# shmurthy08/MoE-GAN_CPSC541

Hardware: AMD Instinct MI355X
Metric: images/sec (G+D step, 64x64 MS-COCO layout) (higher is better)
Workload: dtype bf16; 1 GPU; C2: 64x64, 8 experts top-2, batch 256/GPU, bf16, R1 on; global_batch=256, experts=8, topk=2, parallelism=dp1, world_seen=1, launch=hipGraph replay

## Files before the change

include/moegan_hip.h:

```cpp
#ifndef MOEGAN_HIP_H
#define MOEGAN_HIP_H
#include <stddef.h>
#include <stdint.h>

#ifdef __cplusplus
extern "C" {
#endif

#define MG_OK 0
#define MG_ERR_ARG (-1)
#define MG_ERR_LAUNCH (-2)

#define MG_F32 0
#define MG_BF16 1
#define MG_F32X3 2

#define MG_ACT_NONE 0
#define MG_ACT_LRELU 1
#define MG_ACT_GELU 2
#define MG_ACT_MUL_GELU_GRAD 3
#define MG_ACT_MUL_LRELU_GRAD 4
#define MG_ACT_RSQRT_EPS 5
#define MG_ACT_QUICK_GELU 6
#define MG_ACT_MUL_QUICK_GELU_GRAD 7
// ... 10 lines not shown
  int64_t ld_aux;
  const void* resid;
  int64_t ld_res;
  int32_t accumulate;
  int32_t atomic;
  int32_t remap_lgcin;
  int32_t remap_taps;
  const int32_t* a_idx;
  int32_t a_idx_div;
  const float* a_rowscale;
  int32_t a_gelu;
  const float* addvec;
  int32_t add_shift;
  int64_t add_ld;
  void* out_pre;
  int64_t ld_pre;
  float* gs;
  int64_t gs_ld;
  const void* gs_x;
  int64_t ld_gs_x;
} mg_epilogue;

const char* mg_last_error(void);
int mg_version(void);
const char* mg_source_hash(void);

int mg_set_workspace(void* ptr, size_t bytes, void* stream);
int mg_workspace_reserve(size_t bytes, void* stream);
int64_t mg_workspace_bytes(void* stream);
int mg_set_tuning(int key, int value);

int mg_timer_event_create(void** event);
int mg_timer_event_record(void* event, void* stream);
int mg_timer_event_elapsed(void* start, void* stop, float* ms);
int mg_timer_event_destroy(void* event);
int mg_mark(int tag, void* stream);

typedef struct mg_gemm_desc {
  int32_t M, N, K;
  const void* A;
  int64_t lda;
  const void* B;
  int64_t ldb;
  void* C;
  int64_t ldc;
  const mg_epilogue* ep;
} mg_gemm_desc;

int mg_gemm(int dtype, int M, int N, int K, const void* A, int64_t lda, int a_kc, const void* B, int64_t ldb,
            int b_kc, void* C, int64_t ldc, int c_dtype, const mg_epilogue* ep, int splits, void* stream);

int mg_gemm_batch(int dtype, int a_kc, int b_kc, int c_dtype, int n, const mg_gemm_desc* descs, void* stream);

int mg_conv2d_fwd(int dtype, const void* x, int B, int H, int W, int Cin, const void* wpack, int Cout, int KH,
                  int KW, int stride, int pad, const float* in_scale, void* y, int64_t ldy, int y_dtype,
                  const mg_epilogue* ep, void* stream);

int mg_conv2d_fwd_mx8(const void* x, const void* xscale, int B, int H, int W, int Cin, const void* wq,
                      const void* wscale, int Cout, int KH, int KW, int stride, int pad, void* y, int64_t ldy, int y_dtype, const mg_epilogue* ep,
                      void* stream);

int mg_quant_mx8(const void* x, int64_t ldx, int64_t rows, int K, void* q, void* scale, void* stream);
#define MG_QUANT_BATCH_MAX 32
typedef struct mg_quant_desc {
  const void* x;
  int64_t ldx;
  int64_t rows;
  int32_t K;
  void* q;
  void* scale;
} mg_quant_desc;
int mg_quant_mx8_batch(int n, const mg_quant_desc* d, void* stream);

int mg_conv2d_wgrad(int dtype, const void* gy, int64_t ldg, const void* x, int B, int H, int W, int Cin,
                    const float* in_scale, int Cout, int KH, int KW, int stride, int pad, float* gw, int splits,
                    void* stream);

int mg_conv2d_dgrad_s2(int dtype, const void* g, int B, int OH, int OW, int Cg, const void* wcls, int Cin,
                       void* out, int64_t ldo, int out_dtype, const mg_epilogue* ep, void* stream);

int mg_gemm_grouped(int dtype, int total_rows, int N, int K, int ngroups, const int32_t* row_off,
                    const int32_t* tile_off, int max_tiles, const void* A, int64_t lda, const void* B,
                    int64_t ldb, int b_kc, int64_t b_gstride, void* C, int64_t ldc, int c_dtype,
                    const mg_epilogue* ep, void* stream);

int mg_gemm_grouped_wgrad(int dtype, int M, int N, int ngroups, const int32_t* row_off, int total_rows,
                          const void* A, int64_t lda, const void* B, int64_t ldb, const int32_t* b_idx,
                          int b_idx_div, int b_gelu, float* C, int splits, const mg_epilogue* ep, void* stream);

int mg_moe_ffn_fwd(int dtype, int total_rows, int C, int Hd, int ngroups, const int32_t* row_off, const int32_t* tile_off, int max_tiles, const void* X, int64_t ldx, const int32_t* x_idx, int x_idx_div, const void* W1, const float* b1, const void* W2, const float* b2, void* pre, void* hid, void* Y, void* stream);

int mg_moe_ffn_bwd(int dtype, int total_rows, int C, int Hd, int ngroups, const int32_t* row_off, const int32_t* tile_off, int max_tiles, const void* gG, const void* pre, const void* W1, const void* W2, void* gP, void* gX, void* hid, float* gb1, float* gb2, void* stream);


int mg_clip_patches(int dtype, const void* img, int B, int R, int ld, int res, int patch, void* out, void* stream);

int mg_clip_patches_bwd(int g_dtype, const void* g_patches, int img_dtype, const void* img, int B, int R, int ld, int res, int patch, float alpha, int accumulate, void* g_img, void* stream);

int mg_cos_loss(const float* f, const float* text, int B, int C, const float* scale, float* loss, float* g_f, void* stream);

int mg_layernorm_fwd(int dtype, const void* x, int64_t ldx, int R, int C, const float* gamma, const float* beta, float eps, void* y, int64_t ldy, float* mean, float* rstd, int act, void* stream);

int mg_layernorm_bwd(int dtype, int gy_dtype, const void* gy, int64_t ldg, const void* x, int64_t ldx, int R, int C, const float* mean, const float* rstd, const float* gamma, void* gx, int64_t ldgx, int accumulate, float* ggamma, float* gbeta, void* stream);

int mg_attn_fwd(int dtype, const void* qkv, int B, int L, int C, int heads, void* out, float* lse, void* stream);

// ... 235 lines not shown
```

moe-gan_cpsc541_amd/csrc/mg_common.h:

```cpp
#pragma once
#include <hip/hip_runtime.h>
#include <stdint.h>

#include <algorithm>
#include <atomic>
#include <string>

#include "../../include/moegan_hip.h"

typedef uint16_t bf16_t;
typedef __bf16 bf16x8_t __attribute__((ext_vector_type(8)));
typedef unsigned short u16x8_t __attribute__((ext_vector_type(8)));
typedef unsigned short u16x4_t __attribute__((ext_vector_type(4)));
typedef float f32x4_t __attribute__((ext_vector_type(4)));

#define MG_DEV __device__ __forceinline__

MG_DEV float bf2f(bf16_t h) { return __uint_as_float(((uint32_t)h) << 16); }
MG_DEV bf16_t f2bf(float f) { return __builtin_bit_cast(bf16_t, (__bf16)f); }

MG_DEV float ldf(const float* p, int64_t i) { return p[i]; }
MG_DEV float ldf(const bf16_t* p, int64_t i) { return bf2f(p[i]); }
MG_DEV void stf(float* p, int64_t i, float v) { p[i] = v; }
MG_DEV void stf(bf16_t* p, int64_t i, float v) { p[i] = f2bf(v); }
// ... 76 lines not shown
  const V p = t * q;
  return gcopysign(gfma(-p, g, gsplat<V>(1.f)), x);
}
template <typename V> MG_DEV V gelu_fast_t(V x) {
  V g;
  const V e = gelu_erf_core(x, g);
  const V hx = x * gsplat<V>(0.5f);
  return gfma(hx, e, hx);
}
template <typename V> MG_DEV V gelu_fast_grad_t(V x) {
  V g;
  const V e = gelu_erf_core(x, g);
  return gfma(x * gsplat<V>(0.3989422804014327f), g, gfma(gsplat<V>(0.5f), e, gsplat<V>(0.5f)));
}
MG_DEV float gelu_fast(float x) { return gelu_fast_t<float>(x); }
MG_DEV float gelu_fast_grad(float x) { return gelu_fast_grad_t<float>(x); }
MG_DEV f32x2_t gelu_fast2(f32x2_t x) { return gelu_fast_t<f32x2_t>(x); }
MG_DEV f32x2_t gelu_fast_grad2(f32x2_t x) { return gelu_fast_grad_t<f32x2_t>(x); }

MG_DEV float wave_sum(float v) {
#pragma unroll
  for (int o = 32; o > 0; o >>= 1) v += __shfl_xor(v, o, 64);
  return v;
}
MG_DEV float wave_max(float v) {
#pragma unroll
  for (int o = 32; o > 0; o >>= 1) v = fmaxf(v, __shfl_xor(v, o, 64));
  return v;
}

void mg_set_error(const std::string& msg);
int mg_check_launch(const char* what);
enum { MG_TUNE_WGRAD_TILE = 0, MG_TUNE_GWGRAD_TILE = 1, MG_TUNE_CONV_TILE = 2, MG_TUNE_GEMM_TILE = 3,
       MG_TUNE_WGRAD_SPLITS = 4, MG_TUNE_NO_SLABS = 5, MG_TUNE_XCD = 6 , MG_TUNE_WGRAD_MODE = 7,
       MG_TUNE_WARP_LDS = 8, MG_TUNE_SHORTK = 9, MG_TUNE_ATOMIC_BLOCKS = 10, MG_TUNE_DETERMINISTIC = 11,
       MG_TUNE_S1_OFF = 12,
       MG_TUNE_D0_STORE = 13,
       MG_TUNE_FFN_BWD_OCC = 14,
       MG_TUNE_WIDE_WGRAD = 15,
       MG_TUNE_NARROW = 16,
       MG_TUNE_NARROW_BLOCKS = 17,
       MG_TUNE_DISPATCH3 = 18,
       MG_TUNE_NARROW_WPX = 19,
       MG_TUNE_GWGRAD_BLOCKS = 20,
       MG_TUNE_BATCH_SPLIT = 21,
       MG_TUNE_GROUPED_SHORTK = 22,
       MG_TUNE_SPLITK_FUSED = 23,
       MG_TUNE_ROUTER_TEAM = 24,
       MG_TUNE_ADAMW_CACHED = 25,
       MG_TUNE_ATOMIC_MINK = 26,
       MG_TUNE_WIDE_BLOCKS = 27,
       MG_TUNE_WGRAD_SLAB_BLOCKS = 28,
       MG_TUNE_MODGRAD_UNFUSED = 29,
       MG_TUNE_COUNT = 30 };
extern std::atomic<int> g_mg_tune[MG_TUNE_COUNT];
inline bool mg_det() { return g_mg_tune[MG_TUNE_DETERMINISTIC].load(std::memory_order_relaxed) != 0; }
void* mg_workspace(size_t bytes, hipStream_t stream);
int* mg_tile_counters(int n, hipStream_t stream);
void* mg_fold_alloc(size_t bytes, hipStream_t stream);
int mg_fold_rows_submit(const mg_fold_rows& r, bool deferred, hipStream_t stream);
int mg_fold_wgrad_submit(const mg_fold_wgrad& r, bool deferred, hipStream_t stream);
inline float* mg_fold_partials(size_t bytes, hipStream_t st, bool* deferred) {
  void* p = mg_fold_alloc(bytes, st);
  *deferred = p != nullptr;
  return reinterpret_cast<float*>(p ? p : mg_workspace(bytes, st));
}

namespace {
__global__ __launch_bounds__(1024) void k_det_fold_rows(const float* __restrict__ part, int nrows, int ncols, int na,
                                                        float* __restrict__ out_a, float* __restrict__ out_b) {
  __shared__ float red[16][64];
  const int cx = threadIdx.x & 63, ry = threadIdx.x >> 6;
  const int i = blockIdx.x * 64 + cx;
  float s = 0.f;
  if (i < ncols)
    for (int r = ry; r < nrows; r += 16) s += part[(int64_t)r * ncols + i];
  red[ry][cx] = s;
  __syncthreads();
  if (ry == 0 && i < ncols) {
    float t = 0.f;
#pragma unroll
    for (int y = 0; y < 16; ++y) t += red[y][cx];
    if (i < na) out_a[i] += t;
    else out_b[i - na] += t;
  }
}
__global__ __launch_bounds__(256) void k_det_sum(const float* __restrict__ part, int n, float* __restrict__ out) {
  __shared__ float ws[4];
  float s = 0.f;
  for (int i = threadIdx.x; i < n; i += blockDim.x) s += part[i];
#pragma unroll
  for (int o = 32; o > 0; o >>= 1) s += __shfl_xor(s, o, 64);
  if ((threadIdx.x & 63) == 0) ws[threadIdx.x >> 6] = s;
  __syncthreads();
  if (threadIdx.x == 0) out[0] += (ws[0] + ws[1]) + (ws[2] + ws[3]);
}
}
static inline void mg_det_fold_rows(const float* part, int nrows, int ncols, int na, float* out_a, float* out_b,
                             hipStream_t st) {
  hipLaunchKernelGGL(k_det_fold_rows, dim3((ncols + 63) / 64), dim3(1024), 0, st, part, nrows, ncols, na, out_a, out_b);
}

#define MG_REQUIRE(cond, msg)                       \
  do {                                              \
    if (!(cond)) {                                  \
      mg_set_error(std::string(__func__) + ": " + (msg)); \
      return MG_ERR_ARG;                            \
    }                                               \
  } while (0)

static inline int cdiv(int64_t a, int64_t b) { return (int)((a + b - 1) / b); }

bool mg_conv3_direct_ok(int H, int W, int Cin, int Cout, int KH, int KW, int stride, int pad, bool wgrad);
bool mg_conv3_direct(const void* x, int B, int H, int Cin, const void* wpack, int Cout, const mg_epilogue* e, void* y,
                     int64_t ldy, int y_dtype, hipStream_t st);
bool mg_wgrad3_direct(const void* gy, int64_t ldg, const void* x, int B, int H, int Cin, float** ws_out, int* splits,
                      bool* deferred,
                      hipStream_t st);

int mg_modgrad_gemm(int dtype, int M, int N, int K, const void* A, int64_t lda, const void* B, int64_t ldb, void* C,
                    int64_t ldc, int c_dtype, const mg_epilogue* e, hipStream_t st);
int mg_modgrad_conv(int dtype, const void* x, int B, int H, int W, int Cin, const void* wpack, int Cout, void* y,
                    int64_t ldy, int y_dtype, const mg_epilogue* e, hipStream_t st);

bool mg_wgrad_wide(int M, int N, int K, const void* A, int64_t lda, const void* B, int64_t ldb, float* C, int64_t ldc,
                   float alpha, hipStream_t st);
```

moe-gan_cpsc541_amd/csrc/mg_gemm.hip:

```cpp
#include <algorithm>
#include <string>
#include <type_traits>

#include "mg_gemm.h"
#include "mg_host.h"

using namespace mg;

namespace {


constexpr Grouping kNoGroup{0, 1, nullptr, nullptr, 0};
inline Grouping xcd_group() {
  Grouping g = kNoGroup;
  const int x = g_mg_tune[MG_TUNE_XCD];
  g.swz = x == 0 ? 1 : x == 3 ? 0 : x;
  return g;
}

inline bool a_xf(const mg_epilogue* e) { return e && (e->a_idx || e->a_rowscale || e->a_gelu); }

template <typename T, typename TO, int BM, int BN, bool AK, bool BKc, bool XF, bool X3 = false>
void run_plain(int M, int N, int K, const void* A, int64_t lda, const void* B, int64_t ldb, void* C, int64_t ldc,
               const mg_epilogue* e, int splits, hipStream_t st) {
// ... 113 lines not shown
                         grid, dim3(NTHREADS), 0, st, la, lb, slab, M, N, K, kchunk, xcd_group());
  };
  const T* Ap = reinterpret_cast<const T*>(A);
  const T* Bp = reinterpret_cast<const T*>(B);
  using TT = std::true_type;
  using FF = std::false_type;
  if (a_kc) {
    LdKC<T> la{Ap, lda, M, K, nullptr, 1, nullptr, 0};
    if (b_kc) go(la, LdKC<T>{Bp, ldb, N, K, nullptr, 1, nullptr, 0}, TT{}, TT{});
    else go(la, LdMC<T>{Bp, ldb, N, K, nullptr, 1, nullptr, 0}, TT{}, FF{});
  } else {
    LdMC<T> la{Ap, lda, M, K, nullptr, 1, nullptr, 0};
    if (b_kc) go(la, LdKC<T>{Bp, ldb, N, K, nullptr, 1, nullptr, 0}, FF{}, TT{});
    else go(la, LdMC<T>{Bp, ldb, N, K, nullptr, 1, nullptr, 0}, FF{}, FF{});
  }
  if (cnt) return true;
  int blocks = (int)std::min<int64_t>(cdiv(MN, 256), 2048);
  hipLaunchKernelGGL((splitk_reduce_kernel<Epi<TO>>), dim3(blocks), dim3(256), 0, st, ws, splits, M, N, ep);
  return true;
}

}

extern "C" int mg_gemm(int dtype, int M, int N, int K, const void* A, int64_t lda, int a_kc, const void* B,
                       int64_t ldb, int b_kc, void* C, int64_t ldc, int c_dtype, const mg_epilogue* ep, int splits,
                       void* stream) {
  MG_REQUIRE(dtype == MG_F32 || dtype == MG_BF16 || dtype == MG_F32X3, "bad dtype");
  MG_REQUIRE(M >= 0 && N >= 0 && K >= 0, "negative size");
  if (M == 0 || N == 0) return MG_OK;
  const bool qgg = ep && ep->act == MG_ACT_MUL_QUICK_GELU_GRAD;
  MG_REQUIRE(!qgg || (dtype == MG_BF16 && c_dtype == MG_BF16 && a_kc && !b_kc && splits <= 1 && ep->aux &&
                      !ep->bias && !ep->scale && !ep->out_pre && !ep->atomic && !ep->remap_taps && !a_xf(ep)),
             "MG_ACT_MUL_QUICK_GELU_GRAD: bf16 g [M,K] x W [K,N] -> bf16 with aux, no bias / scale / out_pre / atomic");
  const bool x3 = dtype == MG_F32X3;
  if (x3) dtype = MG_F32;
  const int vec = dtype == MG_F32 ? 4 : 8;
  MG_REQUIRE(aligned16(A) && aligned16(B), "A/B must be 16-byte aligned");
  MG_REQUIRE(lda % vec == 0 && ldb % vec == 0, "lda/ldb must be multiples of the 16-byte vector");
  MG_REQUIRE(a_kc ? (K % vec == 0) : (M % vec == 0), "A vector dim must be a multiple of the 16-byte vector");
  MG_REQUIRE(b_kc ? (K % vec == 0) : (N % vec == 0), "B vector dim must be a multiple of the 16-byte vector");
  MG_REQUIRE(under2g((a_kc ? (int64_t)M : K) * lda, dtype) && under2g((b_kc ? (int64_t)N : K) * ldb, dtype) &&
                 under2g((int64_t)M * ldc, c_dtype),
             "an operand exceeds 2 GiB (32-bit buffer offsets)");
  if (ep && ep->gs) {
    MG_REQUIRE(a_kc && !b_kc && !x3 && splits <= 1, "mg_epilogue.gs: gyt [M, K] x W [K, N], bf16 or fp32, no split-K");
    return mg_modgrad_gemm(dtype, M, N, K, A, lda, B, ldb, C, ldc, c_dtype, ep, reinterpret_cast<hipStream_t>(stream));
  }
  if (splits < 1 && dtype == MG_BF16 && !x3 && !a_kc && !b_kc && c_dtype == MG_F32 && ep && ep->atomic &&
      !ep->bias && !ep->scale && !ep->rowscale && !ep->act && !ep->aux && !ep->resid && !ep->accumulate &&
      !ep->remap_taps && !ep->a_idx && !ep->a_rowscale && !ep->a_gelu && !ep->addvec && !ep->out_pre &&
      mg_wgrad_wide(M, N, K, A, lda, B, ldb, reinterpret_cast<float*>(C), ldc, ep->alpha,
                    reinterpret_cast<hipStream_t>(stream)))
    return mg_check_launch("mg_gemm (wide weight gradient)");
  if (splits < 1) {
    if (ep && ep->atomic) {
      int64_t tiles = (int64_t)cdiv(M, 64) * cdiv(N, 64);
      const int target = g_mg_tune[MG_TUNE_ATOMIC_BLOCKS] > 0 ? (int)g_mg_tune[MG_TUNE_ATOMIC_BLOCKS] : 512;
      int64_t want = std::max<int64_t>(1, target / std::max<int64_t>(tiles, 1));
      const int mink = g_mg_tune[MG_TUNE_ATOMIC_MINK] > 0 ? (int)g_mg_tune[MG_TUNE_ATOMIC_MINK] : 256;
      splits = (int)std::max<int64_t>(1, std::min<int64_t>(want, K / mink));
    } else {
      splits = 1;
    }
  }
  MG_REQUIRE(splits == 1 || (ep && ep->atomic && c_dtype == MG_F32), "split-K requires an atomic fp32 epilogue");
  MG_REQUIRE(!(ep && ep->atomic) || c_dtype == MG_F32, "atomic epilogue requires fp32 C");
  if (K == 0) splits = 1;
  hipStream_t st = reinterpret_cast<hipStream_t>(stream);
  if (splits > 1 && mg_det()) {
    bool done;
    if (x3)
      done = run_splitk_slabs<float, float, true>(a_kc, b_kc, M, N, K, A, lda, B, ldb, C, ldc, ep, st, splits);
    else if (dtype == MG_F32)
      done = run_splitk_slabs<float, float>(a_kc, b_kc, M, N, K, A, lda, B, ldb, C, ldc, ep, st, splits);
    else
      done = run_splitk_slabs<bf16_t, float>(a_kc, b_kc, M, N, K, A, lda, B, ldb, C, ldc, ep, st, splits);
    if (done) return mg_check_launch("mg_gemm (deterministic split-K slabs)");
    splits = 1;
  }
  if (splits == 1 && !(ep && ep->atomic) && !qgg && !g_mg_tune[MG_TUNE_NO_SLABS]) {
    bool done;
    if (x3)
      done = c_dtype == MG_F32 ? run_splitk_slabs<float, float, true>(a_kc, b_kc, M, N, K, A, lda, B, ldb, C, ldc, ep, st)
                               : run_splitk_slabs<float, bf16_t, true>(a_kc, b_kc, M, N, K, A, lda, B, ldb, C, ldc, ep, st);
    else if (dtype == MG_F32)
      done = c_dtype == MG_F32 ? run_splitk_slabs<float, float>(a_kc, b_kc, M, N, K, A, lda, B, ldb, C, ldc, ep, st)
                               : run_splitk_slabs<float, bf16_t>(a_kc, b_kc, M, N, K, A, lda, B, ldb, C, ldc, ep, st);
    else
      done = c_dtype == MG_F32 ? run_splitk_slabs<bf16_t, float>(a_kc, b_kc, M, N, K, A, lda, B, ldb, C, ldc, ep, st)
                               : run_splitk_slabs<bf16_t, bf16_t>(a_kc, b_kc, M, N, K, A, lda, B, ldb, C, ldc, ep, st);
    if (done) return mg_check_launch("mg_gemm (split-K slabs)");
  }
  if (x3) {
    if (c_dtype == MG_F32) run_plain_tiles<float, float, true>(a_kc, b_kc, M, N, K, A, lda, B, ldb, C, ldc, ep, splits, st);
    else run_plain_tiles<float, bf16_t, true>(a_kc, b_kc, M, N, K, A, lda, B, ldb, C, ldc, ep, splits, st);
  } else if (dtype == MG_F32) {
    if (c_dtype == MG_F32) run_plain_tiles<float, float>(a_kc, b_kc, M, N, K, A, lda, B, ldb, C, ldc, ep, splits, st);
    else run_plain_tiles<float, bf16_t>(a_kc, b_kc, M, N, K, A, lda, B, ldb, C, ldc, ep, splits, st);
  } else {
    if (c_dtype == MG_F32) run_plain_tiles<bf16_t, float>(a_kc, b_kc, M, N, K, A, lda, B, ldb, C, ldc, ep, splits, st);
    else run_plain_tiles<bf16_t, bf16_t>(a_kc, b_kc, M, N, K, A, lda, B, ldb, C, ldc, ep, splits, st);
  }
  return mg_check_launch("mg_gemm");
}

namespace {
// ... 56 lines not shown
      r.n = used;
      float* ws = reinterpret_cast<float*>(mg_workspace((size_t)std::max<int64_t>(off, 8) * sizeof(float), st));
      if (ws) {
        args.ws = ws;
        r.ws = ws;
        hipLaunchKernelGGL((gemm_batch_kernel<T, AK, BKc, AL, BL, TO, X3, true>), dim3(tiles, S), dim3(NTHREADS), 0, st,
                           args);
        hipLaunchKernelGGL((batch_reduce_kernel<TO>), dim3(blks), dim3(256), 0, st, r);
        continue;
      }
    }
    hipLaunchKernelGGL((gemm_batch_kernel<T, AK, BKc, AL, BL, TO, X3>), dim3(tiles), dim3(NTHREADS), 0, st, args);
  }
  return mg_check_launch("mg_gemm_batch");
}
}

extern "C" int mg_gemm_batch(int dtype, int a_kc, int b_kc, int c_dtype, int n, const mg_gemm_desc* d,
                             void* stream) {
  MG_REQUIRE(dtype == MG_F32 || dtype == MG_BF16 || dtype == MG_F32X3, "bad dtype");
  const int vec = dtype == MG_BF16 ? 8 : 4;
  const int mdt = dtype == MG_F32X3 ? MG_F32 : dtype;
  for (int i = 0; i < n; ++i) {
    const mg_gemm_desc& q = d[i];
    MG_REQUIRE(q.M >= 0 && q.N >= 0 && q.K >= 0, "negative size");
    MG_REQUIRE(aligned16(q.A) && aligned16(q.B), "A/B must be 16-byte aligned");
    MG_REQUIRE(q.lda % vec == 0 && q.ldb % vec == 0, "lda/ldb must be multiples of the 16-byte vector");
    MG_REQUIRE(a_kc ? (q.K % vec == 0) : (q.M % vec == 0), "A vector dim must be a multiple of the vector");
    MG_REQUIRE(b_kc ? (q.K % vec == 0) : (q.N % vec == 0), "B vector dim must be a multiple of the vector");
    MG_REQUIRE(!(q.ep && q.ep->atomic) || c_dtype == MG_F32, "atomic epilogue requires fp32 C");
    MG_REQUIRE(!a_xf(q.ep), "A loader transforms (a_idx / a_rowscale / a_gelu) are not supported by mg_gemm_batch");
    MG_REQUIRE(!q.ep || q.ep->act != MG_ACT_MUL_QUICK_GELU_GRAD, "MG_ACT_MUL_QUICK_GELU_GRAD: mg_gemm only");
    MG_REQUIRE(under2g((a_kc ? (int64_t)q.M : q.K) * q.lda, mdt) &&
                   under2g((b_kc ? (int64_t)q.N : q.K) * q.ldb, mdt) && under2g((int64_t)q.M * q.ldc, c_dtype),
               "an operand exceeds 2 GiB (32-bit buffer offsets)");
  }
  if (n <= 0) return MG_OK;
  hipStream_t st = reinterpret_cast<hipStream_t>(stream);
  if (mg_det() && n > 1) {
    bool atomic = false;
    for (int i = 0; i < n; ++i) atomic = atomic || (d[i].ep && d[i].ep->atomic);
    if (atomic) {
      for (int i = 0; i < n; ++i) {
        int rc = mg_gemm_batch(dtype, a_kc, b_kc, c_dtype, 1, d + i, stream);
        if (rc) return rc;
      }
      return MG_OK;
    }
  }
#define B_(T, TO, ...)                                                                                          \
  (a_kc ? (b_kc ? run_batch<T, TO, true, true, ##__VA_ARGS__>(n, d, st) : run_batch<T, TO, true, false, ##__VA_ARGS__>(n, d, st)) \
        : (b_kc ? run_batch<T, TO, false, true, ##__VA_ARGS__>(n, d, st) : run_batch<T, TO, false, false, ##__VA_ARGS__>(n, d, st)))
  if (dtype == MG_F32) return c_dtype == MG_F32 ? B_(float, float) : B_(float, bf16_t);
  if (dtype == MG_F32X3) return c_dtype == MG_F32 ? B_(float, float, true) : B_(float, bf16_t, true);
  return c_dtype == MG_F32 ? B_(bf16_t, float) : B_(bf16_t, bf16_t);
#undef B_
}

namespace {
template <typename T, typename TO, int BM, int BN, bool XF = false, bool SC = false>
void run_conv(const void* x, int B, int H, int W, int Cin, const void* wpack, int Cout, int KH, int KW, int stride,
              int pad, const float* sc, void* y, int64_t ldy, const mg_epilogue* e, hipStream_t st) {
  int OH = (H + 2 * pad - KH) / stride + 1, OW = (W + 2 * pad - KW) / stride + 1;
  int M = B * OH * OW, K = KH * KW * Cin;
  LdKCConv<T, XF, SC> la{reinterpret_cast<const T*>(x), H, W, Cin, ilog2(Cin), ilog2(OW), ilog2(OH * OW), M,
                         KW, stride, pad, K, sc, kwinv(KW)};
  LdKC<T> lb{reinterpret_cast<const T*>(wpack), K, Cout, K, nullptr, 1, nullptr, 0};
  auto ep = make_epi<TO>(y, ldy, e);
  launch_gemm<T, BM, BN, true, true>(la, lb, ep, M, Cout, K, 1, kNoGroup, 0, st);
}
template <typename T, typename TO, bool SC, int BM, int BN>
bool conv_slabs_t(const void* x, int B, int H, int W, int Cin, const void* wpack, int Cout, int KH, int KW,
                  int stride, int pad, const float* sc, void* y, int64_t ldy, const mg_epilogue* e, hipStream_t st) {
  constexpr int TBK = tile_bk<T, false, BM, BN>();
  int OH = (H + 2 * pad - KH) / stride + 1, OW = (W + 2 * pad - KW) / stride + 1;
  int M = B * OH * OW, K = KH * KW * Cin;
  int64_t tiles = (int64_t)cdiv(M, BM) * cdiv(Cout, BN);
  const int ksteps = K / TBK;
  if (tiles >= 1024 || ksteps < 16 || (e && e->atomic) || sc || g_mg_tune[MG_TUNE_NO_SLABS]) return false;
  int splits = (int)std::min<int64_t>(cdiv(1024, tiles), ksteps / 8);
  if (splits < 2) return false;
  int kchunk = ((K + splits - 1) / splits + TBK - 1) / TBK * TBK;
  splits = (K + kchunk - 1) / kchunk;
  const int64_t MN = (int64_t)M * Cout;
  float* ws = reinterpret_cast<float*>(mg_workspace((size_t)splits * MN * sizeof(float), st));
  if (!ws) return false;
  mg_epilogue raw{};
  raw.alpha = 1.f;
  Epi<float> slab = make_epi<float>(ws, Cout, &raw);
  slab.zstride = MN;
  slab.vec_ok = slab.host_vec_ok() ? 1 : 0;
  LdKCConv<T, false, SC> la{reinterpret_cast<const T*>(x), H, W, Cin, ilog2(Cin), ilog2(OW), ilog2(OH * OW), M,
                            KW, stride, pad, K, sc, kwinv(KW)};
  LdKC<T> lb{reinterpret_cast<const T*>(wpack), K, Cout, K, nullptr, 1, nullptr, 0};
  dim3 grid(cdiv(M, BM), cdiv(Cout, BN), splits);
  auto ep = make_epi<TO>(y, ldy, e);
  ep.vec_ok = ep.host_vec_ok() ? 1 : 0;
  int* cnt = g_mg_tune[MG_TUNE_SPLITK_FUSED] == 1 ? mg_tile_counters((int)tiles, st) : nullptr;
  if (cnt) {
    hipLaunchKernelGGL((gemm_splitk_fused_kernel<T, BM, BN, true, true, LdKCConv<T, false, SC>, LdKC<T>, TO>), grid,
                       dim3(NTHREADS), 0, st, la, lb, slab, ep, M, Cout, K, kchunk, cnt);
    return true;
  }
  hipLaunchKernelGGL((gemm_kernel<T, BM, BN, true, true, LdKCConv<T, false, SC>, LdKC<T>, Epi<float>>), grid,
                     dim3(NTHREADS), 0, st, la, lb, slab, M, Cout, K, kchunk, xcd_group());
  int blocks = (int)std::min<int64_t>(cdiv(MN, 256), 2048);
// ... 417 lines not shown
```

moe-gan_cpsc541_amd/moegan_mi/roofline.py:

```python
import re

import torch

from . import _lib as L

ELT = {0: 4, 1: 2, 2: 4}
MX8_PEAK_TFLOPS = 5000.0

FAMILIES = {
    "conv_fwd": ("mfma", ("mg_conv2d_fwd",)),
    "conv_fwd_mx8": ("mfma8", ("mg_conv2d_fwd_mx8",)),
    "conv_dgrad_s2": ("mfma", ("mg_conv2d_dgrad_s2",)),
    "conv_wgrad+fold": ("mfma", ("mg_conv2d_wgrad",)),
    "expert_gemm": ("mfma", ("mg_gemm_grouped", "mg_gemm_grouped_wgrad", "mg_moe_ffn_fwd", "mg_moe_ffn_bwd")),
    "gemm": ("mfma", ("mg_gemm", "mg_gemm_batch")),
    "attention": ("mfma", ("mg_attn_fwd", "mg_attn_bwd", "mg_xattn_fwd", "mg_xattn_bwd", "mg_xattn_ragged_fwd",
                          "mg_xattn_ragged_bwd")),
    "router_fwd": ("hbm", ("mg_router_fwd",)),
    "dispatch_combine": ("hbm", ("mg_gather_rows", "mg_moe_combine")),
    "warp_fwd": ("hbm", ("mg_warp_fwd", "mg_warp_fwd_scaled")),
    "mtm_bwd": ("hbm", ("mg_mtm_bwd_fused",)),
    "modconv_bwd_io": ("hbm", ("mg_modconv_bwd_in", "mg_modconv_bwd_out", "mg_scale_bc")),
    "r1": ("hbm", ("mg_r1",)),
    "sumsq": ("hbm", ("mg_sumsq", "mg_grad_norm_steps")),
    "adamw": ("hbm", ("mg_adamw_dev", "mg_adamw_dev_shadow", "mg_adamw_dev_ema", "mg_adamw")),
    "bias_colsum": ("hbm", ("mg_colsum", "mg_grouped_colsum", "mg_colsum_batch", "mg_segsum", "mg_const_bwd")),
    "weight_prep": ("hbm", ("mg_pack_conv", "mg_pack_conv_flip", "mg_pack_dgrad_s2", "mg_wsq", "mg_wsq_bwd",
                            "mg_router_reparam", "mg_weight_norm_fwd", "mg_weight_norm_bwd", "mg_weight_norm_batch",
                            "mg_quant_mx8",
                            "mg_prep_batch")),
    "layernorm": ("hbm", ("mg_layernorm_fwd", "mg_layernorm_bwd")),
    "router_aux": ("hbm", ("mg_router_bwd", "mg_moe_gate_grad", "mg_moe_token_grad", "mg_router_feat_grad",
                           "mg_router_param_bwd", "mg_router_param_bwd_batch", "mg_moe_dispatch", "mg_router_kl",
                           "mg_router_kl_batch")),
    "im2col_col2im": ("hbm", ("mg_im2col_4x4s2", "mg_col2im_4x4s2")),
    "grad_fold": ("hbm", ("mg_fold_flush", "mg_fold_rows_batch", "mg_fold_rows_queue", "mg_fold_defer")),
    "d_conv0": ("hbm", ("mg_d0_fwd", "mg_d0_wgrad", "mg_d0_dgrad")),
    "elementwise": ("hbm", ("mg_cast", "mg_copy2d", "mg_lrelu_mask_mul", "mg_upsample2x_fwd", "mg_upsample2x_bwd",
                            "mg_const_fwd", "mg_gated_axpy", "mg_select_if", "mg_zero_if", "mg_clip_patches",
                            "mg_clip_patches_bwd")),
    "disc_head": ("hbm", ("mg_disc_head_fwd", "mg_disc_head_gmat", "mg_disc_head_sum", "mg_disc_head_bwd_data",
                          "mg_d_head_fwd", "mg_d_head_bwd",
                          "mg_disc_head_bwd_w", "mg_d_text_bwd")),
    "mtm_bwd_unfused": ("hbm", ("mg_warp_bwd", "mg_offset_head_bwd")),
    "losses_flags": ("hbm", ("mg_d_loss", "mg_g_loss", "mg_finite_flag", "mg_flag_window", "mg_kl_coefs", "mg_balance",
                             "mg_opt_prologue", "mg_guard_update", "mg_cos_loss")),
}
_FAMILY_OF = {e: f for f, (_, es) in FAMILIES.items() for e in es}

KERNELS = [
    (r"k_fold_wgrad_batch|k_fold_rows_batch", "grad_fold"),
    (r"k_wgrad_fold|splitk_reduce_kernel<mg::Epi<float>|k_wgrad3_direct", "conv_wgrad+fold"),
    (r"k_conv3_direct", "conv_fwd"),
    (r"k_mx8_conv", "conv_fwd_mx8"),
    (r"gemm_kernel<.*, 1(, (true|false))?>\(|k_moe_ffn_fwd|k_moe_ffn_bwd|k_ffn_bias_fold", "expert_gemm"),
    (r"gemm_kernel<[^>]*LdKCConvT", "conv_dgrad_s2"),
    (r"gemm_kernel<.*LdMCConv", "conv_wgrad+fold"),
    (r"gemm_kernel<.*LdKCConv", "conv_fwd"),
    (r"gemm_kernel<|gemm_batch_kernel<|splitk_reduce_kernel", "gemm"),
    (r"k_attn_|k_xattn_", "attention"),
    (r"k_router_fwd", "router_fwd"),
    (r"k_gather_rows|k_combine", "dispatch_combine"),
    (r"k_warp_fwd", "warp_fwd"),
    (r"k_mtm_bwd", "mtm_bwd"),
    (r"k_bwd_in|k_bwd_out|k_scale_bc", "modconv_bwd_io"),
    (r"k_r1", "r1"),
    (r"k_sumsq", "sumsq"),
    (r"k_adamw", "adamw"),
    (r"k_colsum|k_grouped_colsum|k_segsum|k_const_bwd", "bias_colsum"),
    (r"k_pack_|k_wsq|k_reparam|k_wn_|k_quant_mx8|k_prep_batch", "weight_prep"),
    (r"k_ln_|k_layernorm", "layernorm"),
    (r"k_router_bwd|k_fold_partials|k_gate_grad|k_token_grad|k_router_feat_grad|k_feat_grad_fin|k_router_param_bwd|"
     r"k_disp_|k_router_kl", "router_aux"),
    (r"k_im2col|k_col2im", "im2col_col2im"),
    (r"k_d0_|k_fold_cols", "d_conv0"),
    (r"k_wgrad_wide|k_wide_fold|k_wide_final", "gemm"),
    (r"k_cast|k_copy2d|k_mask_mul|k_up2|k_const_fwd|k_gated_axpy|k_select_if|k_zero_if|k_clip_patches",
     "elementwise"),
    (r"k_head_|k_d_text|k_dhead_", "disc_head"),
    (r"k_warp_bwd|k_offset_head", "mtm_bwd_unfused"),
    (r"k_d_loss|k_g_loss|k_finite_flag|k_flag_window|k_guard_update|k_kl_coefs|k_balance|k_opt_prologue|"
     r"k_cos_loss",
     "losses_flags"),
]


def kernel_family(kernel_name):
    for pat, fam in KERNELS:
        if re.search(pat, kernel_name):
            return fam
    return "other"


def _conv_out(H, W, KH, KW, s, p):
    return (H + 2 * p - KH) // s + 1, (W + 2 * p - KW) // s + 1


def work(name, a):
    if name in ("mg_conv2d_fwd", "mg_conv2d_wgrad", "mg_conv2d_fwd_mx8"):
        OH, OW = _conv_out(a["H"], a["W"], a["KH"], a["KW"], a["stride"], a["pad"])
        return 2.0 * a["B"] * OH * OW * a["Cout"] * a["KH"] * a["KW"] * a["Cin"]
    if name == "mg_conv2d_dgrad_s2":
        return 2.0 * a["B"] * (2 * a["OH"]) * (2 * a["OW"]) * a["Cin"] * a["Cg"] * 4
    if name == "mg_gemm":
        return 2.0 * a["M"] * a["N"] * a["K"]
    if name == "mg_gemm_batch":
        d = a["descs"]
        return sum(2.0 * d[i].M * d[i].N * d[i].K for i in range(a["n"]))
    if name == "mg_gemm_grouped":
        return 2.0 * a["total_rows"] * a["N"] * a["K"]
    if name == "mg_gemm_grouped_wgrad":
        return 2.0 * a["M"] * a["N"] * a["total_rows"]
# ... 359 lines not shown
```

Measured before the change: 32650 images/sec.

## Add small-M fp32x3 GEMM kernel with 32x32 tiles and in-block split-K

Adds a dedicated kernel for small fp32-emulated (bf16x3 split) GEMMs with M up to 512. It uses 32x32 tiles, a four-stage register prefetch pipeline, and waves that each take a slice of K and are reduced through shared memory. Both single and batched GEMM paths route to it when the shape and epilogue allow, with a tune flag to turn it off. The aim is more parallelism and less split-K reduction overhead on small router and head GEMMs. The cost is another code path whose epilogue support is limited, and it may lose to the existing tiled kernels on some shapes.

Result: no change. 32810 images/sec, median of 4 (+0.5%).

```diff
diff --git a/include/moegan_hip.h b/include/moegan_hip.h
--- a/include/moegan_hip.h
+++ b/include/moegan_hip.h
@@ -86,6 +86,8 @@
 
 int mg_gemm_batch(int dtype, int a_kc, int b_kc, int c_dtype, int n, const mg_gemm_desc* descs, void* stream);
 
+int mg_gemm_rows_fusable(int dtype, int M, int N, int K, const void* A, int64_t lda, int a_kc, const void* B, int64_t ldb, int b_kc, const void* C, int64_t ldc, int c_dtype, const mg_epilogue* ep, int splits);
+
 int mg_conv2d_fwd(int dtype, const void* x, int B, int H, int W, int Cin, const void* wpack, int Cout, int KH,
                   int KW, int stride, int pad, const float* in_scale, void* y, int64_t ldy, int y_dtype,
                   const mg_epilogue* ep, void* stream);
diff --git a/moe-gan_cpsc541_amd/csrc/mg_common.h b/moe-gan_cpsc541_amd/csrc/mg_common.h
--- a/moe-gan_cpsc541_amd/csrc/mg_common.h
+++ b/moe-gan_cpsc541_amd/csrc/mg_common.h
@@ -152,7 +152,8 @@
        MG_TUNE_WIDE_BLOCKS = 27,
        MG_TUNE_WGRAD_SLAB_BLOCKS = 28,
        MG_TUNE_MODGRAD_UNFUSED = 29,
-       MG_TUNE_COUNT = 30 };
+       MG_TUNE_ROWS_OFF = 30,
+       MG_TUNE_COUNT = 31 };
 extern std::atomic<int> g_mg_tune[MG_TUNE_COUNT];
 inline bool mg_det() { return g_mg_tune[MG_TUNE_DETERMINISTIC].load(std::memory_order_relaxed) != 0; }
 void* mg_workspace(size_t bytes, hipStream_t stream);
@@ -223,5 +224,8 @@
 int mg_modgrad_conv(int dtype, const void* x, int B, int H, int W, int Cin, const void* wpack, int Cout, void* y,
                     int64_t ldy, int y_dtype, const mg_epilogue* e, hipStream_t st);
 
+bool mg_rows_batch_ok(int dtype, int a_kc, int b_kc, int c_dtype, int n, const mg_gemm_desc* d);
+void mg_rows_launch(int b_kc, int c_dtype, int n, const mg_gemm_desc* d, bool batched, hipStream_t st);
+
 bool mg_wgrad_wide(int M, int N, int K, const void* A, int64_t lda, const void* B, int64_t ldb, float* C, int64_t ldc,
                    float alpha, hipStream_t st);
diff --git a/moe-gan_cpsc541_amd/csrc/mg_gemm.hip b/moe-gan_cpsc541_amd/csrc/mg_gemm.hip
--- a/moe-gan_cpsc541_amd/csrc/mg_gemm.hip
+++ b/moe-gan_cpsc541_amd/csrc/mg_gemm.hip
@@ -189,6 +189,11 @@
       mg_wgrad_wide(M, N, K, A, lda, B, ldb, reinterpret_cast<float*>(C), ldc, ep->alpha,
                     reinterpret_cast<hipStream_t>(stream)))
     return mg_check_launch("mg_gemm (wide weight gradient)");
+  if (x3 && mg_gemm_rows_fusable(MG_F32X3, M, N, K, A, lda, a_kc, B, ldb, b_kc, C, ldc, c_dtype, ep, splits)) {
+    const mg_gemm_desc q{M, N, K, A, lda, B, ldb, C, ldc, ep};
+    mg_rows_launch(b_kc, c_dtype, 1, &q, false, reinterpret_cast<hipStream_t>(stream));
+    return mg_check_launch("mg_gemm (batch rows)");
+  }
   if (splits < 1) {
     if (ep && ep->atomic) {
       int64_t tiles = (int64_t)cdiv(M, 64) * cdiv(N, 64);
@@ -351,6 +356,22 @@
   (a_kc ? (b_kc ? run_batch<T, TO, true, true, ##__VA_ARGS__>(n, d, st) : run_batch<T, TO, true, false, ##__VA_ARGS__>(n, d, st)) \
         : (b_kc ? run_batch<T, TO, false, true, ##__VA_ARGS__>(n, d, st) : run_batch<T, TO, false, false, ##__VA_ARGS__>(n, d, st)))
   if (dtype == MG_F32) return c_dtype == MG_F32 ? B_(float, float) : B_(float, bf16_t);
+  if (dtype == MG_F32X3 && a_kc && g_mg_tune[MG_TUNE_ROWS_OFF] != 1) {
+    for (int i0 = 0; i0 < n; i0 += MG_BATCH_MAX) {
+      const int cnt = std::min(MG_BATCH_MAX, n - i0);
+      const mg_gemm_desc* dc = d + i0;
+      if (mg_rows_batch_ok(dtype, a_kc, b_kc, c_dtype, cnt, dc)) {
+        mg_rows_launch(b_kc, c_dtype, cnt, dc, true, st);
+        continue;
+      }
+      const int rc = b_kc ? (c_dtype == MG_F32 ? run_batch<float, float, true, true, true>(cnt, dc, st)
+                                               : run_batch<float, bf16_t, true, true, true>(cnt, dc, st))
+                          : (c_dtype == MG_F32 ? run_batch<float, float, true, false, true>(cnt, dc, st)
+                                               : run_batch<float, bf16_t, true, false, true>(cnt, dc, st));
+      if (rc) return rc;
+    }
+    return mg_check_launch("mg_gemm_batch (batch rows)");
+  }
   if (dtype == MG_F32X3) return c_dtype == MG_F32 ? B_(float, float, true) : B_(float, bf16_t, true);
   return c_dtype == MG_F32 ? B_(bf16_t, float) : B_(bf16_t, bf16_t);
 #undef B_
diff --git a/moe-gan_cpsc541_amd/csrc/mg_rows.hip b/moe-gan_cpsc541_amd/csrc/mg_rows.hip
--- /dev/null
+++ b/moe-gan_cpsc541_amd/csrc/mg_rows.hip
@@ -0,0 +1,316 @@
+#include <algorithm>
+
+#include "mg_gemm.h"
+#include "mg_host.h"
+
+using namespace mg;
+
+namespace {
+
+constexpr int RW_BM = 32, RW_BN = 32;
+constexpr int RW_DEPTH = 4;
+constexpr int RW_MAXW = 8;
+constexpr int RW_PITCH = RW_BN + 4;
+constexpr int RW_MAX_M = 512;
+constexpr int64_t RW_MAX_WORK = (int64_t)1 << 27;
+
+template <typename TO>
+struct RowsArgs {
+  const float* A[MG_BATCH_MAX];
+  const float* B[MG_BATCH_MAX];
+  int64_t lda[MG_BATCH_MAX], ldb[MG_BATCH_MAX];
+  Epi<TO> e[MG_BATCH_MAX];
+  int M[MG_BATCH_MAX], N[MG_BATCH_MAX], K[MG_BATCH_MAX], tiles_m[MG_BATCH_MAX], tile_off[MG_BATCH_MAX + 1];
+  int per[MG_BATCH_MAX];
+  int n, total;
+};
+
+MG_DEV float bload1(rsrc_t r, uint32_t voff, uint32_t soff) {
+  return __builtin_bit_cast(float, __builtin_amdgcn_raw_buffer_load_b32(r, voff, soff, 0));
+}
+
+MG_DEV void split8(const float* v, bf16x8_t& hi, bf16x8_t& lo) {
+  u16x8_t h, l;
+#pragma unroll
+  for (int j = 0; j < 8; ++j) {
+    h[j] = f2bf(v[j]);
+    l[j] = f2bf(v[j] - bf2f(h[j]));
+  }
+  hi = __builtin_bit_cast(bf16x8_t, h);
+  lo = __builtin_bit_cast(bf16x8_t, l);
+}
+
+template <bool B_KC, typename TO>
+__global__ __launch_bounds__(RW_MAXW * 64) void gemm_rows_kernel(RowsArgs<TO> args) {
+  extern __shared__ __attribute__((aligned(16))) float rw_part[];
+  const int per8 = (args.total + 7) >> 3;
+  const int t = (blockIdx.x & 7) * per8 + (blockIdx.x >> 3);
+  if (t >= args.total) return;
+  int p = 0;
+  while (p + 1 < args.n && t >= args.tile_off[p + 1]) ++p;
+  const int lt = t - args.tile_off[p];
+  const int tn = lt / args.tiles_m[p], tm = lt - tn * args.tiles_m[p];
+  const int m0 = tm * RW_BM, n0 = tn * RW_BN;
+  const int M = args.M[p], N = args.N[p], K = args.K[p];
+  const int W = blockDim.x >> 6;
+  const int wave = __builtin_amdgcn_readfirstlane(threadIdx.x >> 6), lane = threadIdx.x & 63;
+  const int fq = lane >> 4, fr = lane & 15;
+
+  const int steps = (K + 31) >> 5, per = args.per[p];
+  const int s_beg = wave * per, s_end = min(steps, s_beg + per);
+  const int nact = min(W, (steps + per - 1) / per);
+
+  const rsrc_t rA = make_rsrc(args.A[p]), rB = make_rsrc(args.B[p]);
+  const int lda = (int)args.lda[p], ldb = (int)args.ldb[p];
+  uint32_t aoff[2], boff[2];
+#pragma unroll
+  for (int f = 0; f < 2; ++f) {
+    const int r = m0 + f * 16 + fr;
+    aoff[f] = r < M ? (uint32_t)(((int64_t)r * lda + fq * 8) * 4) : MG_OOB;
+    const int c = n0 + f * 16 + fr;
+    if constexpr (B_KC) boff[f] = c < N ? (uint32_t)(((int64_t)c * ldb + fq * 8) * 4) : MG_OOB;
+    else boff[f] = c < N ? (uint32_t)(((int64_t)fq * 8 * ldb + c) * 4) : MG_OOB;
+  }
+
+  float ra[RW_DEPTH][2][8], rb[RW_DEPTH][2][8];
+  auto issue = [&](auto R, int s) {
+    constexpr int r = decltype(R)::value;
+    const int klim = s < s_end ? K : 0;
+    const int k0 = s << 5, kl = k0 + fq * 8;
+    const uint32_t sa = (uint32_t)k0 * 4u;
+#pragma unroll
+    for (int f = 0; f < 2; ++f)
+#pragma unroll
+      for (int h = 0; h < 2; ++h) {
+        const f32x4_t v = bload<f32x4_t>(rA, (kl + 4 * h < klim) ? aoff[f] + 16u * h : MG_OOB, sa);
+#pragma unroll
+        for (int j = 0; j < 4; ++j) ra[r][f][4 * h + j] = v[j];
+      }
+    if constexpr (B_KC) {
+#pragma unroll
+      for (int f = 0; f < 2; ++f)
+#pragma unroll
+        for (int h = 0; h < 2; ++h) {
+          const f32x4_t v = bload<f32x4_t>(rB, (kl + 4 * h < klim) ? boff[f] + 16u * h : MG_OOB, sa);
+#pragma unroll
+          for (int j = 0; j < 4; ++j) rb[r][f][4 * h + j] = v[j];
+        }
+    } else {
+      const uint32_t sb = (uint32_t)k0 * (uint32_t)ldb * 4u;
+#pragma unroll
+      for (int f = 0; f < 2; ++f)
+#pragma unroll
+        for (int j = 0; j < 8; ++j)
+          rb[r][f][j] = bload1(rB, (kl + j < klim) ? boff[f] + (uint32_t)j * (uint32_t)ldb * 4u : MG_OOB, sb);
+    }
+  };
+
+  f32x4_t acc[2][2];
+#pragma unroll
+  for (int i = 0; i < 2; ++i)
+#pragma unroll
+    for (int j = 0; j < 2; ++j) acc[i][j] = f32x4_t{0.f, 0.f, 0.f, 0.f};
+  auto consume = [&](auto R) {
+    constexpr int r = decltype(R)::value;
+    bf16x8_t ah[2], al[2], bh[2], bl[2];
+#pragma unroll
+    for (int f = 0; f < 2; ++f) {
+      split8(ra[r][f], ah[f], al[f]);
+      split8(rb[r][f], bh[f], bl[f]);
+    }
+#pragma unroll
+    for (int i = 0; i < 2; ++i)
+#pragma unroll
+      for (int j = 0; j < 2; ++j) {
+        acc[i][j] = __builtin_amdgcn_mfma_f32_16x16x32_bf16(al[i], bh[j], acc[i][j], 0, 0, 0);
+        acc[i][j] = __builtin_amdgcn_mfma_f32_16x16x32_bf16(ah[i], bl[j], acc[i][j], 0, 0, 0);
+        acc[i][j] = __builtin_amdgcn_mfma_f32_16x16x32_bf16(ah[i], bh[j], acc[i][j], 0, 0, 0);
+      }
+  };
+
+  using I0 = std::integral_constant<int, 0>;
+  using I1 = std::integral_constant<int, 1>;
+  using I2 = std::integral_constant<int, 2>;
+  using I3 = std::integral_constant<int, 3>;
+  static_assert(RW_DEPTH == 4, "the stage rotation below is written out for four stages");
+  issue(I0{}, s_beg);
+  __builtin_amdgcn_sched_barrier(0);
+  issue(I1{}, s_beg + 1);
+  __builtin_amdgcn_sched_barrier(0);
+  issue(I2{}, s_beg + 2);
+  __builtin_amdgcn_sched_barrier(0);
+  issue(I3{}, s_beg + 3);
+  __builtin_amdgcn_sched_barrier(0);
+  for (int s = s_beg; s < s_end; s += RW_DEPTH) {
+    if (s + RW_DEPTH < s_end) {
+      consume(I0{});
+      __builtin_amdgcn_sched_barrier(0);
+      issue(I0{}, s + 4);
+      __builtin_amdgcn_sched_barrier(0);
+      consume(I1{});
+      __builtin_amdgcn_sched_barrier(0);
+      issue(I1{}, s + 5);
+      __builtin_amdgcn_sched_barrier(0);
+      consume(I2{});
+      __builtin_amdgcn_sched_barrier(0);
+      issue(I2{}, s + 6);
+      __builtin_amdgcn_sched_barrier(0);
+      consume(I3{});
+      __builtin_amdgcn_sched_barrier(0);
+      issue(I3{}, s + 7);
+      __builtin_amdgcn_sched_barrier(0);
+    } else {
+      consume(I0{});
+      __builtin_amdgcn_sched_barrier(0);
+      if (s + 1 < s_end) consume(I1{});
+      __builtin_amdgcn_sched_barrier(0);
+      if (s + 2 < s_end) consume(I2{});
+      __builtin_amdgcn_sched_barrier(0);
+      if (s + 3 < s_end) consume(I3{});
+    }
+  }
+
+  if (wave < nact) {
+    float* mine = rw_part + wave * (RW_BM * RW_PITCH);
+#pragma unroll
+    for (int i = 0; i < 2; ++i)
+#pragma unroll
+      for (int j = 0; j < 2; ++j)
+#pragma unroll
+        for (int q = 0; q < 4; ++q) mine[(i * 16 + fq * 4 + q) * RW_PITCH + j * 16 + fr] = acc[i][j][q];
+  }
+  __syncthreads();
+  const Epi<TO>& ep = args.e[p];
+  for (int e = threadIdx.x; e < RW_BM * (RW_BN / 8); e += blockDim.x) {
+    const int r = e >> 2, c = (e & 3) * 8;
+    const int m = m0 + r, n = n0 + c;
+    if (m < M && n < N) {
+      float v[8] = {0.f, 0.f, 0.f, 0.f, 0.f, 0.f, 0.f, 0.f};
+      for (int w = 0; w < nact; ++w) {
+        const float* src = rw_part + w * (RW_BM * RW_PITCH) + r * RW_PITCH + c;
+        const f32x4_t x = *reinterpret_cast<const f32x4_t*>(src), y = *reinterpret_cast<const f32x4_t*>(src + 4);
+#pragma unroll
+        for (int j = 0; j < 4; ++j) {
+          v[j] += x[j];
+          v[j + 4] += y[j];
+        }
+      }
+      if (ep.vec_ok && (N & 7) == 0) {
+        ep.vec8(m, n, v);
+      } else {
+#pragma unroll
+        for (int j = 0; j < 8; ++j)
+          if (n + j < N) ep(m, n + j, v[j]);
+      }
+    }
+  }
+}
+
+int rows_slices(int M, int N, int K, bool batched, int* per) {
+  const int steps = cdiv(K, 32);
+  const int64_t tiles = (int64_t)cdiv(M, 64) * cdiv(N, 64);
+  int splits = 1;
+  if (!batched && tiles < 96 && K >= 256) splits = (int)std::min<int64_t>(256 / tiles, K / 128);
+  if (splits < 2) {
+    *per = std::max(steps, 1);
+    return 1;
+  }
+  const int kchunk = cdiv(cdiv(K, splits), 64) * 64;
+  splits = cdiv(K, kchunk);
+  *per = kchunk / 32;
+  return splits <= RW_MAXW ? splits : 0;
+}
+
+bool rows_epilogue_ok(const mg_epilogue* e, int c_dtype) {
+  if (!e) return true;
+  if (e->rowscale || e->remap_taps || e->a_idx || e->a_rowscale || e->a_gelu || e->addvec || e->out_pre || e->gs)
+    return false;
+  if (e->act != MG_ACT_NONE && e->act != MG_ACT_LRELU && e->act != MG_ACT_RSQRT_EPS &&
+      !(e->act == MG_ACT_MUL_LRELU_GRAD && e->aux))
+    return false;
+  if (e->atomic && c_dtype != MG_F32) return false;
+  return true;
+}
+
+bool rows_ok(int dtype, int M, int N, int K, const void* A, int64_t lda, int a_kc, const void* B, int64_t ldb, int b_kc,
+             const void* C, int64_t ldc, int c_dtype, const mg_epilogue* e, bool batched) {
+  if (g_mg_tune[MG_TUNE_ROWS_OFF] == 1) return false;
+  if (dtype != MG_F32X3 || !a_kc) return false;
+  if (c_dtype != MG_F32 && c_dtype != MG_BF16) return false;
+  if (M <= 0 || N <= 0 || K <= 0 || M > RW_MAX_M || !A || !B || !C) return false;
+  if ((int64_t)M * N * K > RW_MAX_WORK) return false;
+  int per;
+  if (!rows_slices(M, N, K, batched, &per)) return false;
+  if (!aligned16(A) || !aligned16(B) || lda % 4 || ldb % 4 || K % 4 || (!b_kc && N % 4)) return false;
+  if (lda < K || ldb < (b_kc ? K : N) || ldc < N) return false;
+  if (!under2g((int64_t)M * lda, MG_F32) || !under2g((b_kc ? (int64_t)N : K) * ldb, MG_F32) ||
+      !under2g((int64_t)M * ldc, c_dtype))
+    return false;
+  return rows_epilogue_ok(e, c_dtype);
+}
+
+template <bool B_KC, typename TO>
+void rows_launch_t(int n, const mg_gemm_desc* d, bool batched, hipStream_t st) {
+  RowsArgs<TO> args;
+  static_assert(sizeof(args) <= 4096, "kernel arguments over 4 KB");
+  int used = 0, tiles = 0, W = 1;
+  for (int j = 0; j < n; ++j) {
+    const mg_gemm_desc& q = d[j];
+    if (q.M == 0 || q.N == 0) continue;
+    args.A[used] = reinterpret_cast<const float*>(q.A);
+    args.B[used] = reinterpret_cast<const float*>(q.B);
+    args.lda[used] = q.lda;
+    args.ldb[used] = q.ldb;
+    args.e[used] = make_epi<TO>(q.C, q.ldc, q.ep);
+    args.e[used].vec_ok = args.e[used].host_vec_ok() ? 1 : 0;
+    args.M[used] = q.M;
+    args.N[used] = q.N;
+    args.K[used] = q.K;
+    args.tiles_m[used] = cdiv(q.M, RW_BM);
+    args.tile_off[used] = tiles;
+    tiles += cdiv(q.M, RW_BM) * cdiv(q.N, RW_BN);
+    W = std::max(W, rows_slices(q.M, q.N, q.K, batched, &args.per[used]));
+    ++used;
+  }
+  if (!used) return;
+  args.tile_off[used] = tiles;
+  args.n = used;
+  args.total = tiles;
+  hipLaunchKernelGGL((gemm_rows_kernel<B_KC, TO>), dim3(8 * cdiv(tiles, 8)), dim3(W * 64),
+                     (size_t)W * RW_BM * RW_PITCH * sizeof(float), st, args);
+}
+
+}
+
+extern "C" int mg_gemm_rows_fusable(int dtype, int M, int N, int K, const void* A, int64_t lda, int a_kc,
+                                    const void* B, int64_t ldb, int b_kc, const void* C, int64_t ldc, int c_dtype,
+                                    const mg_epilogue* ep, int splits) {
+  if (splits > 1 && !(ep && ep->atomic)) return 0;
+  return rows_ok(dtype, M, N, K, A, lda, a_kc, B, ldb, b_kc, C, ldc, c_dtype, ep, false) ? 1 : 0;
+}
+
+bool mg_rows_batch_ok(int dtype, int a_kc, int b_kc, int c_dtype, int n, const mg_gemm_desc* d) {
+  if (n <= 0 || n > MG_BATCH_MAX) return false;
+  if (!b_kc) return false;
+  bool any = false;
+  int64_t work = 0;
+  for (int j = 0; j < n; ++j) {
+    const mg_gemm_desc& q = d[j];
+    if (q.M == 0 || q.N == 0) continue;
+    work += (int64_t)q.M * q.N * q.K;
+    if (work > RW_MAX_WORK) return false;
+    if (!rows_ok(dtype, q.M, q.N, q.K, q.A, q.lda, a_kc, q.B, q.ldb, b_kc, q.C, q.ldc, c_dtype, q.ep, true)) return false;
+    any = true;
+  }
+  return any;
+}
+
+void mg_rows_launch(int b_kc, int c_dtype, int n, const mg_gemm_desc* d, bool batched, hipStream_t st) {
+  if (b_kc) {
+    if (c_dtype == MG_F32) rows_launch_t<true, float>(n, d, batched, st);
+    else rows_launch_t<true, bf16_t>(n, d, batched, st);
+  } else {
+    if (c_dtype == MG_F32) rows_launch_t<false, float>(n, d, batched, st);
+    else rows_launch_t<false, bf16_t>(n, d, batched, st);
+  }
+}
diff --git a/moe-gan_cpsc541_amd/moegan_mi/roofline.py b/moe-gan_cpsc541_amd/moegan_mi/roofline.py
--- a/moe-gan_cpsc541_amd/moegan_mi/roofline.py
+++ b/moe-gan_cpsc541_amd/moegan_mi/roofline.py
@@ -57,7 +57,7 @@
     (r"gemm_kernel<[^>]*LdKCConvT", "conv_dgrad_s2"),
     (r"gemm_kernel<.*LdMCConv", "conv_wgrad+fold"),
     (r"gemm_kernel<.*LdKCConv", "conv_fwd"),
-    (r"gemm_kernel<|gemm_batch_kernel<|splitk_reduce_kernel", "gemm"),
+    (r"gemm_kernel<|gemm_batch_kernel<|gemm_rows_kernel<|splitk_reduce_kernel", "gemm"),
     (r"k_attn_|k_xattn_", "attention"),
     (r"k_router_fwd", "router_fwd"),
     (r"k_gather_rows|k_combine", "dispatch_combine"),
```
